# pierluigiferrari/fcn8s_tensorflow

Hardware: AMD Instinct MI355X
Metric: training images/sec at 1024x512 bs16 (higher is better)
Workload: dtype f32; 1 GPU; FCN-8s (VGG-16, fc6 7x7, 20 classes) train step, 1024x512, 16 images/GPU, SGD+momentum, keep_prob 0.5; global_batch=16, parallelism=dp1

## Files before the change

### fcn8s_tensorflow_amd/csrc/fcn8s_internal.h

```cpp
#pragma once
#include <hip/hip_runtime.h>
#include <stdint.h>
#include "../../include/fcn8s_hip.h"

#if defined(__HIP_DEVICE_COMPILE__) && !defined(__gfx950__)
#error "libfcn8s_hip is written for gfx950 (MI355X) only: build with --offload-arch=gfx950"
#endif
#define FCN8S_LDS_BYTES_NEEDED (160u * 1024u)

#include <string>
namespace fcn8s {

extern thread_local const char* g_last_kernel;
void defer_error(int code, const char* fmt, ...) __attribute__((format(printf, 2, 3)));
int take_deferred_error(std::string* text);

struct IgemmArgs {
    const float* x; const float* w; const float* bias; const float* addend; const float* mask;
    float* y;
    int N, Ma, Mb; long long M;
    int Hi, Wi, Cin, ldx;
    int KW, in_scale, tap_step, tap_off, Ktot;
    int Ho, Wo, Cout, ldy;
    int out_scale, out_offy, out_offx;
    int phases_x; long long w_phase_stride;
    float alpha; int relu; float mask_scale;
    int dropout; float keep_prob; unsigned long long seed; unsigned int stream_id;
    int batched; long long x_batch_stride, y_batch_stride;
    int m_fastest;
    int bt, ldw;
    int fixed_tile;
    int split;
};
void launch_igemm(const IgemmArgs& a, int phases, hipStream_t s);

struct Bf16ConvArgs {
    const float* x; const unsigned short* xh;
    const unsigned short* wt; const float* bias; float* y;
    int N, H, W, Cin, Cout, K;
    int relu, dropout; float keep_prob; unsigned long long seed; unsigned int stream_id;
    long long M; int m_fastest;
};
void launch_w_to_bf16_tiles(const float* w, unsigned short* wt, int K, int Cout, hipStream_t s);
bool launch_conv_bf16(const Bf16ConvArgs& a, hipStream_t s);
void launch_f32_to_bf16(const float* x, unsigned short* y, long long n, hipStream_t s);
struct Bf16Conv256Args {
    const unsigned short* xp; const unsigned short* wt; const float* bias; float* y;
    int N, H, W, Cin, Cout, K;
    int relu, dropout; float keep_prob; unsigned long long seed; unsigned int stream_id;
    long long M; int m_fastest;
    const float* addend;
    const float* mask; float mask_scale;
    int any_shape;
    const unsigned short* mask16;
    float* colpart;
    int ksplit; float* part;
    int rows_bn;
    int guarded;
    unsigned short* yb; int yb_pad;
    long long xp_ps, yb_ps, mask16_ps;
};
bool conv_bf16_256_ok(long long M, int Cin, int Cout, int mode);
void launch_w_to_bf16_t(const float* w, unsigned short* wt, int K, int Cout, hipStream_t s);
void launch_f32_to_bf16_padded(const float* x, unsigned short* xp, int N, int H, int W, int C, int pad, hipStream_t s, long long ps = 0);
int conv_bf16_rows_bm(int Cout, int rows_bn);
bool launch_conv_bf16_256(const Bf16Conv256Args& a, hipStream_t s);
struct Fp8ConvArgs {
// ... 220 lines not shown
```

### fcn8s_tensorflow_amd/csrc/igemm.hip

```cpp
#include "fcn8s_internal.h"
#include <cmath>
#include <cstdlib>
#include <map>
#include <mutex>
#include <string>

namespace fcn8s {

thread_local const char* g_last_kernel = nullptr;
#define FCN8S_STR2(x) #x
#define FCN8S_STR(x) FCN8S_STR2(x)

typedef float f32x16 __attribute__((ext_vector_type(16)));
constexpr int BK_ = 16;

static __device__ __forceinline__ float4 ldg4(const float* p) { return *reinterpret_cast<const float4*>(p); }

static __device__ __forceinline__ unsigned xcd_swizzle(unsigned p, unsigned total)
{
    const unsigned q = total >> 3, r = total & 7u, xcd = p & 7u, i = p >> 3;
    return (xcd < r ? xcd * (q + 1) : r * (q + 1) + (xcd - r) * q) + i;
}

thread_local int t_deterministic = 0;
// ... 604 lines not shown
                    float4 v = *reinterpret_cast<const float4*>(&patch[row * LDT + (lane & 7) * 4]);
                    v.x += bv.x; v.y += bv.y; v.z += bv.z; v.w += bv.w;
                    if (mrow + row < p.M) {
                        if (p.mask) {
                            const float4 mk = ldg4(p.mask + (mrow + row) * p.ldy + n0 + wn * TN * 32 + tn * 32 + (lane & 7) * 4);
                            v.x = mk.x > 0.f ? v.x * p.mask_scale : 0.f; v.y = mk.y > 0.f ? v.y * p.mask_scale : 0.f;
                            v.z = mk.z > 0.f ? v.z * p.mask_scale : 0.f; v.w = mk.w > 0.f ? v.w * p.mask_scale : 0.f;
                        }
                        *reinterpret_cast<float4*>(yb + (mrow + row) * p.ldy) = v;
                    }
                }
                __builtin_amdgcn_wave_barrier();
            }
        return;
    }
#pragma unroll
    for (int tn = 0; tn < TN; ++tn) {
        const int col = n0 + wn * TN * 32 + tn * 32 + (lane & 31);
        const float bv = p.bias ? p.bias[col] : 0.f;
#pragma unroll
        for (int tm = 0; tm < TM; ++tm)
#pragma unroll
            for (int r = 0; r < 16; ++r) {
                const long long m = m0 + wm * TM * 32 + tm * 32 + (r & 3) + 8 * (r >> 2) + 4 * (lane >> 5);
                if (m >= p.M) continue;
                const long long off = m * p.ldy;
                float v = acc[tm][tn][r] * p.alpha + bv;
                if (p.addend) v += p.addend[off + col];
                if (p.relu) v = v > 0.f ? v : 0.f;
                if (p.mask) v = p.mask[off + col] > 0.f ? v * p.mask_scale : 0.f;
                if (p.dropout) v = dropout_apply(v, (unsigned long long)(off + col), p.seed, p.stream_id, p.keep_prob);
                Y[off + col] = v;
            }
    }
}

static __device__ __forceinline__ void glds16v(const float* vaddr, unsigned lds_byte_off)
{
    asm volatile("s_mov_b32 m0, %1\n\ts_nop 0\n\tglobal_load_lds_dwordx4 %0, off" ::"v"(vaddr), "s"(lds_byte_off) : "memory", "m0");
}
struct Conv1Args { const float* x4; const float* w48; const float* bias; float* y; const float* zero16; int N, H, W; long long M;
                   unsigned short* yb16; long long yb16_ps; };

__global__ __launch_bounds__(256, 4) void conv1_glds_kernel(const Conv1Args p)
{
    constexpr int BM = 128, BN = 64, BK = 16, NKT = 3, WN = 2, TM = 2, TN = 1, CH = 4, RPI = 16;
    constexpr int A_PW = BM / RPI / 4;
    constexpr int STAGE = BM * BK + BK * BN;
    __shared__ __attribute__((aligned(16))) float smem[NKT * STAGE];
    const int tid = threadIdx.x, lane = tid & 63, wave = __builtin_amdgcn_readfirstlane(tid >> 6);
    const int wm = wave / WN, wn = wave % WN;
    const long long m0 = (long long)blockIdx.x * BM;
    const unsigned lds0 = (unsigned)(size_t)(__attribute__((address_space(3))) float*)smem;
#pragma unroll
    for (int i = 0; i < A_PW; ++i) {
        const int row = (wave * A_PW + i) * RPI + lane / CH, pc = lane % CH;
        const int c = pc ^ ((row >> 2) & 3);
        long long m = m0 + row; if (m >= p.M) m = p.M - 1;
        const int x = (int)(m % p.W); const long long r = m / p.W; const int y = (int)(r % p.H);
#pragma unroll
        for (int kt = 0; kt < NKT; ++kt) {
            const int t = kt * 4 + c, dy = t / 3 - 1, dx = t % 3 - 1;
            const bool ok = t < 9 && (unsigned)(y + dy) < (unsigned)p.H && (unsigned)(x + dx) < (unsigned)p.W;
            const float* src = ok ? p.x4 + (m + (long long)dy * p.W + dx) * 4 : p.zero16;
            glds16v(src, lds0 + (unsigned)(kt * STAGE + (wave * A_PW + i) * 256) * 4u);
        }
// ... 218 lines not shown
                else if (a.split == 2) hipLaunchKernelGGL((gemm_glds_nt_x2_kernel<BM, BN, WM, WN, 3>), grid, dim3(256), 0, s, a);
                else                   hipLaunchKernelGGL((gemm_glds_nt_kernel<BM, BN, WM, WN, 3>), grid, dim3(256), 0, s, a);
                return;
            }
            g_last_kernel = gt[(epi ? 1 : 0) + (a.split == 3 ? 2 : 0)].c_str();
            if (a.split == 3) {
                if (epi) hipLaunchKernelGGL((gemm_glds_x3_kernel<BM, BN, WM, WN, 3, true>), grid, dim3(256), 0, s, a);
                else     hipLaunchKernelGGL((gemm_glds_x3_kernel<BM, BN, WM, WN, 3, false>), grid, dim3(256), 0, s, a);
                return;
            }
            if (a.split == 2) {
                static const std::string x2base = "gemm_glds_x2_kernel<" + std::to_string(BM) + ", " + std::to_string(BN) + ", " + std::to_string(WM) + ", " + std::to_string(WN) + ", 3, ";
                static const std::string x2t[2] = {x2base + "false>", x2base + "true>"};
                g_last_kernel = x2t[epi ? 1 : 0].c_str();
                if (epi) hipLaunchKernelGGL((gemm_glds_x2_kernel<BM, BN, WM, WN, 3, true>), grid, dim3(256), 0, s, a);
                else     hipLaunchKernelGGL((gemm_glds_x2_kernel<BM, BN, WM, WN, 3, false>), grid, dim3(256), 0, s, a);
                return;
            }
            if (epi) hipLaunchKernelGGL((gemm_glds_kernel<BM, BN, WM, WN, 3, true>), grid, dim3(256), 0, s, a);
            else     hipLaunchKernelGGL((gemm_glds_kernel<BM, BN, WM, WN, 3, false>), grid, dim3(256), 0, s, a);
            return;
        }
    }
    if (a.bt) {
        defer_error(FCN8S_ERR_STATE, "transposed-B GEMM (M %lld, K %d, N %d, tile %dx%d) does not fit the LDS-DMA kernel", a.M, a.Ktot, a.Cout, BM, BN);
        return;
    }
    if (mode == 3)      hipLaunchKernelGGL((igemm_fwd_kernel<BM, BN, WM, WN, 3, BKF>), grid, dim3(256), 0, s, a);
    else if (mode == 2) hipLaunchKernelGGL((igemm_fwd_kernel<BM, BN, WM, WN, 2, BKF>), grid, dim3(256), 0, s, a);
    else if (mode == 1) hipLaunchKernelGGL((igemm_fwd_kernel<BM, BN, WM, WN, 1, BKF>), grid, dim3(256), 0, s, a);
    else                hipLaunchKernelGGL((igemm_fwd_kernel<BM, BN, WM, WN, 0, 16>), grid, dim3(256), 0, s, a);
}

void launch_igemm(const IgemmArgs& a, int phases, hipStream_t s)
{
    auto cost = [&](int bm, int bn, int bpc, double eff) {
        const long long blocks = ((a.M + bm - 1) / bm) * ((a.Cout + bn - 1) / bn) * phases;
        const long long n = (blocks + 255) / 256, rem = n % bpc;
        const double tail = rem == 0 ? 0.0 : (rem == 1 ? 2.0 : (rem == 2 ? 2.4 : 3.0));
        return ((double)(n / bpc) * bpc + tail) * bm * bn / eff;
    };
    if (a.fixed_tile && a.Cout % 128 == 0) { launch_igemm_cfg<128, 128, 2, 2>(a, phases, s); return; }
    if (a.fixed_tile && a.Cout % 64 == 0)  { launch_igemm_cfg<128, 64, 2, 2>(a, phases, s); return; }
    if (a.Cout <= 32)      launch_igemm_cfg<128, 32, 4, 1>(a, phases, s);
    else if (a.Cout <= 64) {
        if (cost(128, 64, 4, 1.0) <= cost(64, 64, 4, 0.9)) launch_igemm_cfg<128, 64, 2, 2>(a, phases, s);
        else                                               launch_igemm_cfg<64, 64, 2, 2>(a, phases, s);
    } else {
        const double c128 = cost(128, 128, 3, 1.0), c64x128 = cost(64, 128, 4, 0.9), c64 = cost(64, 64, 4, 0.85);
        if (a.M > 64 && c128 <= c64x128 && c128 <= c64) launch_igemm_cfg<128, 128, 2, 2>(a, phases, s);
        else if (c64x128 <= c64)                        launch_igemm_cfg<64, 128, 2, 2>(a, phases, s);
        else                                            launch_igemm_cfg<64, 64, 2, 2>(a, phases, s);
    }
}

template <int BM, int BN, int WM, int WN, int WK, bool FAST, bool COLSUM>
__global__ __launch_bounds__(256, FAST ? 4 : 1) void wgrad_kernel(const WgradArgs p, const int chunk)
{
    constexpr int BK = 16, LDA = BM, LDB = BN;
    constexpr int TM = BM / WM / 32, TN = BN / WN / 32;
    constexpr int A_F4 = BK * BM / 4, B_F4 = BK * BN / 4;
    constexpr int A_LD = (A_F4 + 255) / 256, B_LD = (B_F4 + 255) / 256;
    static_assert(WM * WN * WK == 4, "4 waves");
    __shared__ __attribute__((aligned(16))) float smem[2 * BK * LDA + 2 * BK * LDB];
    float* As = smem;
    float* Bs = smem + 2 * BK * LDA;

    const int tid = threadIdx.x, lane = tid & 63, wave = tid >> 6;
// ... 848 lines not shown
```

### fcn8s_tensorflow_amd/csrc/model.hip

```cpp
#include "../../include/fcn8s_hip.h"
#include "fcn8s_internal.h"
#include "device_buffer.h"
#include "pass_state.h"
#include <cstdarg>

#include <dlfcn.h>
#include <atomic>
#include <chrono>
#include <thread>
#include <cmath>
#include <cstdio>
#include <cstring>
#include <cstdlib>
#include <algorithm>
#include <mutex>
#include <map>
#include <set>
#include <string>
#include <vector>

using namespace fcn8s;

extern "C" {
typedef struct ncclComm* ncclComm_t;
// ... 60 lines not shown
    std::map<std::string, int> index;
    size_t total = 0;
    size_t bucket_off[FCN8S_MAX_BUCKETS] = {0}, bucket_n[FCN8S_MAX_BUCKETS] = {0};
    hipEvent_t bucket_ev[FCN8S_MAX_BUCKETS] = {nullptr};
    bool bucket_final[FCN8S_MAX_BUCKETS] = {false};
    ncclComm_t comm = nullptr; int comm_rank = 0, comm_world = 1;
    hipStream_t comm_stream = nullptr;
    static constexpr int kCommSlots = FCN8S_MAX_BUCKETS + 1, kCommMisc = FCN8S_MAX_BUCKETS;
    hipEvent_t comm_done[kCommSlots] = {nullptr}; bool comm_pending[FCN8S_MAX_BUCKETS] = {false};
    std::mutex comm_mu;
    std::thread comm_watch; std::atomic<bool> comm_watch_stop{false}, comm_failed{false};
    std::atomic<bool> comm_inflight[kCommSlots] = {}; int64_t comm_enq_ns[kCommSlots] = {0};
    std::string comm_error; int64_t comm_timeout_ms = 600000;
    float *d_params = nullptr, *d_grads = nullptr;
    DeviceBuf<float> own_params, own_grads;
    DeviceBuf<float> d_m, d_v, d_wt, d_w1pad, d_tph[3];
    DeviceBuf<float> d_wino_u; float *d_wino_v = nullptr, *d_wino_m = nullptr;
    size_t ufl = 0;
    int wino_min_cin = 64;
    int wino_tile = 6;
    int wino_fc6 = 1;
    int fc6_fft = 1;
    int fc6_fft_wgrad = 1;
    int wino_tile_hires = 0, wino_hires_pixels = 0;
    int wino_force_tile = 0;
    int precision = FCN8S_PREC_F32;
    bool frozen = false;
    unsigned long long frozen_fp = 0; DeviceBuf<unsigned long long> d_fp;
    PinnedBuf<unsigned long long> h_fp; hipEvent_t fp_event = nullptr;
    std::map<std::string, DeviceBuf<float>> u_cache;
    std::map<std::string, DeviceBuf<float>> u_train;
    bool fwd_train = false;
    PassState pass;
    int deterministic = 0;
    int fuse_dgrad_dout = 1;
    int fuse_out_in = 1;
    int conv1_tiled = 1, conv1_wgrad_mfma = 1;
    int conv1_in_transform = 1;
    DeviceBuf<unsigned short> d_wbf16;
    std::map<std::string, DeviceBuf<unsigned short>> wbf16_cache;
    std::set<std::string> bank_stale; bool banks_stale = false;
    int bf16_gemm256 = 1;
    DeviceBuf<unsigned short> d_abf16;
    std::map<std::string, DeviceBuf<unsigned short>> xbf16;
    using G16Map = std::map<std::string, DeviceBuf<unsigned short>>;
    G16Map xg16, dyg16;
    std::set<std::string> g16_stale;
    int bf16_fuse_pool = 1;
    int bf16_infer_copies = 1;
    int bf16_rows_bn = 0;
    int bf16_acts = 1;
    bool fp8_calibrated = false, fp8_calibrating = false; float fp8_amax[FCN8S_FP8_LAYERS] = {}; DeviceBuf<unsigned> d_fp8_amax;
    std::map<std::string, Q8Buf> q8;
    std::map<std::string, W8Bank> w8; std::set<std::string> w8_valid;
    int saved_wino_min_cin = -1, saved_wino_fc6 = -1;
    int bf16_copy_by_transform = 1;
    int64_t ws_allocs = 0;
    bool x0_ready = false;
    DeviceBuf<char> crf_buf;
    DeviceBuf<char> tta_buf;
    hipStream_t stream = nullptr;
    int64_t step = 0;
    int N = 0, H = 0, W = 0;
    int plan_N = 0;
    DeviceBuf<char> arena;
    std::map<std::string, Act> acts;
// ... 155 lines not shown
            m->groups[k].ev_shared.emplace_back(a, b);
        }
    }
};

static void prof_derived(fcn8s_model* m, const char* what)
{
    if (m && m->profile && m->profile_detail) m->groups[group_id(m, (std::string("derived:") + what).c_str())].launches += 1;
}

struct ConvEpi { float alpha = 1.f; };
struct FwdEpi : ConvEpi {
    const float* bias = nullptr; int relu = 0;
    int dropout = 0; float keep = 1.f; uint32_t stream_id = 0;
    float* pool_out = nullptr; unsigned char* pool_idx = nullptr;
    int skip_y = 0;
    unsigned* relu_bits_out = nullptr;
    unsigned* in_relu_bits_out = nullptr; const char* in_layer = nullptr;
    float* next_v = nullptr; const char* next_layer = nullptr;
};
struct DgradEpi : ConvEpi {
    const float* addend = nullptr;
    const float* mask = nullptr; float mask_scale = 1.f;
    const unsigned* relu_bits_in = nullptr;
    const float* w_fwd = nullptr;
    int lazy_wt = 0;
    float* dm_out = nullptr; const char* dm_out_layer = nullptr;
    const char* yb_layer = nullptr; int yb_K = 3;
    bool yb_only = false;
};

static bool bt_gemm_ok(int K, int N) { return K % 16 == 0 && (N == 64 || N % 128 == 0); }
thread_local int t_op_split = 0;
thread_local int t_op_rows_bn = 0;
thread_local int t_op_planes = 1;
int split_of(const fcn8s_model* m)
{
    if (!m) return t_op_split;
    if (m->precision == FCN8S_PREC_F32X3 || m->precision == FCN8S_PREC_BF16_FWD) return 3;
    if (m->precision == FCN8S_PREC_F32X2 || m->precision == FCN8S_PREC_BF16_FWD_X2) return 2;
    return 0;
}
static inline bool bf16_fwd_mode(const fcn8s_model* m) { return m->precision == FCN8S_PREC_BF16_FWD || m->precision == FCN8S_PREC_BF16_FWD_X2; }
static inline bool bf16_train_mode(const fcn8s_model* m) { return m && m->precision == FCN8S_PREC_BF16_TRAIN; }
static inline long long bf16_guard_rows(int K, int Wp) { return (long long)((K - 1) / 2) * Wp + (K - 1) / 2 + 640; }
#ifndef A_PLANES
#define A_PLANES 1
#endif
static inline long long g16_ps(int N, int H, int W, int K) { const int pad = (K - 1) / 2, Wp_ = W + 2 * pad; return A_PLANES ? ((long long)N * (H + 2 * pad) * Wp_ + 2 * bf16_guard_rows(K, Wp_)) * 32 : 0; }
static inline long long g16_off(long long G, int C) { return A_PLANES ? G * 32 : G * C; }
unsigned short* g16_for(fcn8s_model* m, fcn8s_model::G16Map& bufs, const char* layer, int N, int H, int W, int C, int K, hipStream_t s);
unsigned short* dyb_for(fcn8s_model* m, const char* layer, const float* dy, int N, int H, int W, int C, int K, hipStream_t s, float* db = nullptr, bool* db_done = nullptr);

int wino_tile_for(const fcn8s_model* m, int H, int W, int K = 3)
{
    if (!m || H % 2 || W % 2) return 0;
    if (m->wino_force_tile && K == 3) return (m->wino_force_tile == 6 || (H % m->wino_force_tile == 0 && W % m->wino_force_tile == 0)) ? m->wino_force_tile : 0;
    int tmax = m->wino_tile;
    if (K == 3 && m->wino_tile_hires && m->wino_hires_pixels > 0 && (long long)H * W >= m->wino_hires_pixels && m->wino_tile_hires < tmax) tmax = m->wino_tile_hires;
    const bool t4 = tmax >= 4 && H % 4 == 0 && W % 4 == 0;
    if (K == 7) return (m->wino_tile >= 4 && H % 4 == 0 && W % 4 == 0) ? 4 : 0;
    if (tmax == 6) {
        auto rows = [&](long long tiles) { return m->plan_N == 1 ? (tiles + 63) / 64 * 64 : tiles; };
        const long long c6 = 64LL * rows((long long)((H + 5) / 6) * ((W + 5) / 6)), c4 = t4 ? 36LL * rows((long long)(H / 4) * (W / 4)) : 16LL * rows((long long)(H / 2) * (W / 2));
        if (c6 < c4) return 6;
    }
    return t4 ? 4 : 2;
}
long long wino_tiles(int tile, int N, int H, int W) { return (long long)N * ((H + tile - 1) / tile) * ((W + tile - 1) / tile); }
struct WinoEpi { const float* bias = nullptr; const float* addend = nullptr; const float* mask = nullptr; float mask_scale = 1.f;
                 int relu = 0; int dropout = 0; float keep = 1.f; unsigned long long seed = 0; unsigned int stream_id = 0; float* pool = nullptr; unsigned char* pidx = nullptr;
                 unsigned* rbits_out = nullptr; const unsigned* rbits_in = nullptr; int skip_y = 0;
                 unsigned* in_rbits_out = nullptr;
                 float* next_v = nullptr; bool* fused_out = nullptr; };
static bool fft6_cheaper(const fcn8s_model* m, int H, int W)
// ... 84 lines not shown
    { ProfScope ps(m, "fc6_fft_transform", 0, 4.0 * ((double)N * H * W * Cout + (double)P * T * Cout)); launch_fft_fc6_dout(dz, m->d_wino_m, N, H, W, Cout, s); }
    m->pass.fft6_dyf.give(layer);
    WgradArgs g{}; g.split = 0;
    g.A = xf; g.B = m->d_wino_m; g.C = m->d_wino_u;
    g.N = 1; g.Pa = 1; g.Pb = (int)T; g.P = T;
    g.Ha = 1; g.Wa = (int)T; g.Adim = Cin; g.lda = Cin; g.Areal = Cin;
    g.Bdim = Cout; g.ldb = Cout; g.KW = 1; g.a_scale = 1; g.tap_off = 0; g.ntaps = P; g.ldc = Cout; g.alpha = 1.f; g.colsum = nullptr;
    g.batched = 1; g.a_batch_stride = wino_slab(T, Cin); g.b_batch_stride = wino_slab(T, Cout); g.c_uninitialized = 1;
    { ProfScope ps(m, "fc6_fft_gemm_wgrad", 2.0 * P * T * Cin * Cout, 4.0 * P * (T * (double)(Cin + Cout) + (double)Cin * Cout), layer); launch_wgrad(g, s); }
    { ProfScope ps(m, "fc6_fft_transform", 0, 4.0 * (P + 49.0) * Cin * Cout); launch_fft_fc6_dfilter(m->d_wino_u, dw, Cin, Cout, s); }
    if (db) { ProfScope ps(m, "colsum", 0, 4.0 * N * H * W * Cout); launch_colsum(dz, db, (long long)N * H * W, Cout, s); }
}
static void conv_fft6_dgrad(fcn8s_model* m, const char* layer, const float* dz, const float* uf, float* dx, int N, int H, int W, int Cin, int Cout, hipStream_t s)
{
    const int P = fft_fc6_planes();
    const long long T = fft_fc6_tiles(N, H, W);
    if (!m->pass.fft6_dyf.take(layer)) {
        m->pass.fft6_dyf.drop();
        ProfScope ps(m, "fc6_fft_transform", 0, 4.0 * ((double)N * H * W * Cin + (double)P * T * Cin)); launch_fft_fc6_dout(dz, m->d_wino_m, N, H, W, Cin, s);
    }
    IgemmArgs a = fft6_gemm(m->d_wino_m, uf, m->d_wino_v, T, Cin, Cout);
    a.fixed_tile = 1; a.bt = 1; a.ldw = Cin;
    { ProfScope ps(m, "fc6_fft_gemm_dgrad", 2.0 * P * T * Cin * Cout, 4.0 * P * (T * (double)(Cin + Cout) + (double)Cin * Cout), layer); launch_igemm(a, P, s); }
    { ProfScope ps(m, "fc6_fft_transform", 0, 4.0 * ((double)P * T * Cout + 2.0 * 196.0 * T * Cout + (double)N * H * W * Cout));
      launch_fft_fc6_din(m->d_wino_v, m->d_wino_m, dx, N, H, W, Cout, s); }
}

void conv_winograd(fcn8s_model* m, int tile, int KS, bool fwd, const float* x, const float* wk, float* y, float* u, float* v, float* mm,
                   int N, int H, int W, int Cin, int Cout, const WinoEpi& e, hipStream_t s, const char* layer, bool v_ready = false)
{
    const int P = wino_alpha(tile, KS) * wino_alpha(tile, KS), nsub2 = wino_nsub(KS) * wino_nsub(KS);
    const long long T = wino_tiles(tile, N, H, W);
    const int Kg = nsub2 * Cin;
    IgemmArgs a = fft6_gemm(v, u, mm, T, Kg, Cout); a.split = split_of(m);
    const double tb = 4.0 * ((double)N * H * W * Cin * nsub2 + (double)P * T * Kg), ob = 4.0 * ((double)N * H * W * Cout * ((e.pool ? (e.skip_y ? 0.25 : 1.25) : 1.0) + (e.rbits_in ? 1.0 / 32 : (e.mask ? 1.0 : 0.0)) + (e.addend ? 1.0 : 0.0) + (e.rbits_out ? 1.0 / 32 : 0.0)) + (double)P * T * Cout);
    bool u_cached = false;
    const char* tag = KS == 7 ? (fwd ? "wino_gemm_fc6_fwd" : "wino_gemm_fc6_dgrad") : (fwd ? "wino_gemm_fwd" : "wino_gemm_dgrad");
    if (m && m->frozen && layer && fwd) {
        DeviceBuf<float>& cu = m->u_cache[std::string(layer) + "#" + std::to_string(tile)];
        const std::string key = "u:" + std::string(layer) + "#" + std::to_string(tile);
        if (cu && !m->bank_stale.count(key)) { u = cu; u_cached = true; }
        else if (cu) { u = cu; m->bank_stale.erase(key); }
        else if (cu.grow((size_t)P * Kg * Cout * sizeof(float), s, &m->ws_allocs)) u = cu;
        a.w = u;
    }
    if (m && !u_cached && m->fwd_train && layer && fwd && ((KS == 3 && tile == 6) || (KS == 7 && tile == 4))) {
        DeviceBuf<float>& tu = m->u_train[std::string(layer) + "#" + std::to_string(tile)];
        if (tu.grow((size_t)P * Kg * Cout * sizeof(float), s)) { u = tu; a.w = u; }
    }
    auto pre = [&]() { if (!u_cached) { prof_derived(m, "wino_filter_kernel"); launch_wino_filter(tile, wk, u, Cin, Cout, KS, s); } if (!v_ready) launch_wino_input(tile, x, v, N, H, W, Cin, KS, s, e.in_rbits_out); };
    auto post = [&]() {
        if (e.next_v && tile == 6 && KS == 3 && e.relu && e.bias && !e.addend && !e.mask && !e.dropout && !e.pool && !e.rbits_in &&
            launch_wino_out_in(mm, e.bias, e.next_v, e.rbits_out, N, H, W, Cout, s, m && m->fuse_out_in >= 2)) { if (e.fused_out) *e.fused_out = true; return; }
        launch_wino_output(tile, mm, e.bias, e.addend, e.mask, e.mask_scale, e.relu, (e.skip_y && e.pool) ? nullptr : y, N, H, W, Cout, e.dropout, e.keep, e.seed, e.stream_id, s, e.pool, e.pidx, KS, e.rbits_out, e.rbits_in); };
    const double ob_fused = 4.0 * (2.0 * P * T * Cout + (e.rbits_out ? (double)N * H * W * Cout / 32 : 0.0));
    { ProfScope ps(m, "wino_transform", 0, (v_ready ? 0.0 : tb) + (u_cached ? 0.0 : (double)(KS * KS + P * nsub2) * 4 * Cin * Cout)); pre(); }
    { ProfScope ps(m, tag, 2.0 * P * T * Kg * Cout, 4.0 * P * (T * (double)(Kg + Cout) + (double)Kg * Cout), layer); launch_igemm(a, P, s); }
    { ProfScope ps(m, "wino_transform", 0, ob); post(); if (e.fused_out && *e.fused_out && m && m->profile && !m->groups.empty()) { const int g = group_id(m, "wino_transform"); m->groups[g].bytes += ob_fused - ob; } }
}

static void conv_direct(fcn8s_model* m, const char* group, IgemmArgs a, const float* x, const float* w, float* y,
                        int N, int H, int W, int Cin, int Cout, int K, hipStream_t s, int real_cin, const char* layer)
{
    a.split = split_of(m);
    a.x = x; a.w = w; a.y = y;
    a.N = N; a.Ma = H; a.Mb = W; a.M = (long long)N * H * W;
    a.Hi = H; a.Wi = W; a.Cin = Cin; a.ldx = Cin;
// ... 76 lines not shown
              done = launch_conv_bf16_256(g, s); }
            if (done) {
                if (g.yb) m->pass.dyg16_filled.insert(e.yb_layer);
                if (g.colpart) {
                    ProfScope ps(m, "colsum", 0, 4.0 * prow * Cout);
                    launch_colsum(g.colpart, Gp(m, std::string(e.yb_layer) + "/biases"), prow, Cout, s);
                    m->pass.db_taken.insert(e.yb_layer); m->pass.dy_bf16_only.insert(e.yb_layer);
                }
                return;
            }
            if (g.colpart) { defer_error(FCN8S_ERR_SHAPE, "bf16_train: %s's data gradient was refused by the flat-position kernel", layer); return; }
        }
    }
    if (bf16_step && m->pass.dy_bf16_only.count(layer)) {
        defer_error(FCN8S_ERR_SHAPE, "bf16_train: %s's data gradient could not run on the bf16 kernel and its fp32 output gradient was not kept (option \"bf16_acts\" = 0 keeps it)", layer); return;
    }
    if (bf16_step && e.mask && m->pass.in_bf16_only.count(layer)) {
        defer_error(FCN8S_ERR_SHAPE, "bf16_train: %s's data gradient could not run on the bf16 kernel and its fp32 mask was not kept (option \"bf16_acts\" = 0 keeps it)", layer); return;
    }
    const bool dm_ready = m && m->pass.dm.take(layer), v_ready = m && m->pass.dgrad_v.take(layer);
    if (m) m->pass.drop_backward_handoffs();
    if (m && K == 7 && layer && e.alpha == 1.f && !e.addend && !e.mask && !e.relu_bits_in) {
        auto kept = m->u_train.find(std::string(layer) + "#fft");
        if (m->pass.fft6_ready.holds(layer) && kept != m->u_train.end() && kept->second && fft6_on(m, N, H, W, Cout, Cin) && bt_gemm_ok(Cin, Cout)) {
            conv_fft6_dgrad(m, layer, x, kept->second, y, N, H, W, Cin, Cout, s);
            return;
        }
    }
    const bool wino3 = m && K == 3 && m->wino_min_cin > 0 && Cin >= m->wino_min_cin && m->d_wino_v && wino_tile_for(m, H, W, 3);
    const bool wino7 = m && K == 7 && m->wino_fc6 && m->d_wino_v && wino_tile_for(m, H, W, 7) == 4;
    if (wino3 && dm_ready && e.w_fwd && wino_tile_for(m, H, W, 3) == 6 && Cin % 64 == 0 && Cout % 64 == 0 && e.alpha == 1.f) {
        const int P = 64;
        const long long T = wino_tiles(6, N, H, W);
        IgemmArgs a = fft6_gemm(m->d_wino_m, m->d_wino_u, m->d_wino_v, T, Cin, Cout); a.split = split_of(m);
        auto kept = m->u_train.find(std::string(layer) + "#6");
        if (kept != m->u_train.end() && kept->second && bt_gemm_ok(Cin, Cout)) {
            a.w = kept->second; a.bt = 1; a.ldw = Cin;
        } else {
            ProfScope ps(m, "wino_transform", 0, (double)(9 + P) * 4 * Cin * Cout); launch_wino_filter(6, e.w_fwd, m->d_wino_u, Cout, Cin, 3, s, 1);
        }
        { ProfScope ps(m, "wino_gemm_dgrad", 2.0 * P * T * Cin * Cout, 4.0 * P * (T * (double)(Cin + Cout) + (double)Cin * Cout), layer); launch_igemm(a, P, s); }
        if (e.dm_out && e.dm_out_layer && e.relu_bits_in && !e.addend && e.mask_scale == 1.f) {
            ProfScope ps(m, "wino_transform", 0, 4.0 * ((double)N * H * W * Cout / 32 + 2.0 * P * T * Cout));
            launch_wino_dgrad_output_dout(m->d_wino_v, e.relu_bits_in, e.dm_out, N, H, W, Cout, s);
            m->pass.dm_prefilled.give(e.dm_out_layer);
            return;
        }
        { ProfScope ps(m, "wino_transform", 0, 4.0 * ((double)N * H * W * Cout * (1.0 + (e.relu_bits_in ? 1.0 / 32 : (e.mask ? 1.0 : 0.0)) + (e.addend ? 1.0 : 0.0)) + (double)P * T * Cout));
          launch_wino_dgrad_output(m->d_wino_v, e.addend, e.mask, e.mask_scale, e.relu_bits_in, y, N, H, W, Cout, s); }
        return;
    }
    if (wino7 && dm_ready && e.alpha == 1.f && !e.mask && !e.addend && bt_gemm_ok(Cin, 4 * Cout)) {
        auto kept = m->u_train.find(std::string(layer) + "#4");
        if (kept != m->u_train.end() && kept->second) {
            const int P = 49, Ng = 4 * Cout;
            const long long T = wino_tiles(4, N, H, W);
            IgemmArgs a = fft6_gemm(m->d_wino_m, kept->second, m->d_wino_v, T, Cin, Ng); a.split = split_of(m);
            a.bt = 1; a.ldw = Cin;
            { ProfScope ps(m, "wino_gemm_fc6_dgrad", 2.0 * P * T * Cin * Ng, 4.0 * P * (T * (double)(Cin + Ng) + (double)Cin * Ng), layer); launch_igemm(a, P, s); }
            { ProfScope ps(m, "wino_transform", 0, 4.0 * ((double)N * H * W * Cout + (double)P * T * Ng)); launch_wino_dgrad_output_sub44(m->d_wino_v, y, N, H, W, Cout, s); }
            return;
        }
    }
    if (e.lazy_wt && e.w_fwd) {
        ProfScope ps(m, "weight_relayout", 0, 8.0 * K * K * Cin * Cout); launch_flip_transpose(e.w_fwd, const_cast<float*>(w), K * K, Cout, Cin, s);
    }
    if ((wino3 || wino7) && Cin % 16 == 0 && Cout % 64 == 0 && e.alpha == 1.f) {
// ... 1366 lines not shown
    if (!m->fp8_calibrated) return FCN8S_ERR_STATE;
    memcpy(amax, m->fp8_amax, sizeof m->fp8_amax);
    return FCN8S_OK;
}
int fcn8s_fp8_set_calibration(fcn8s_model* m, const float* amax, int n)
{
    if (!m || !amax) return fail(m, FCN8S_ERR_BAD_ARG, "fcn8s_fp8_set_calibration: null argument");
    if (n != FCN8S_FP8_LAYERS) return fail(m, FCN8S_ERR_BAD_ARG, "fcn8s_fp8_set_calibration: needs FCN8S_FP8_LAYERS (14) maxima");
    for (int i = 0; i < n; ++i)
        if (!std::isfinite(amax[i]) || amax[i] < 0.f) return fail(m, FCN8S_ERR_BAD_ARG, "fcn8s_fp8_set_calibration: maxima must be finite and >= 0");
    memcpy(m->fp8_amax, amax, sizeof m->fp8_amax);
    m->fp8_calibrated = true;
    return FCN8S_OK;
}

static int* model_option(fcn8s_model* m, const std::string& key)
{
    if (key == "winograd_min_cin") return &m->wino_min_cin;
    if (key == "winograd_tile") return &m->wino_tile;
    if (key == "winograd_fc6") return &m->wino_fc6;
    if (key == "fc6_fft") return &m->fc6_fft;
    if (key == "fc6_fft_wgrad") return &m->fc6_fft_wgrad;
    if (key == "tconv_gemm") return &m->tconv_gemm;
    if (key == "fuse_dgrad_dout") return &m->fuse_dgrad_dout;
    if (key == "fuse_out_in") return &m->fuse_out_in;
    if (key == "bf16_gemm256") return &m->bf16_gemm256;
    if (key == "winograd_tile_hires") return &m->wino_tile_hires;
    if (key == "winograd_hires_pixels") return &m->wino_hires_pixels;
    if (key == "conv1_tiled") return &m->conv1_tiled;
    if (key == "conv1_wgrad_mfma") return &m->conv1_wgrad_mfma;
    if (key == "bf16_copy_by_transform") return &m->bf16_copy_by_transform;
    if (key == "conv1_in_transform") return &m->conv1_in_transform;
    if (key == "deterministic") return &m->deterministic;
    if (key == "bf16_acts") return &m->bf16_acts;
    if (key == "bf16_rows_bn") return &m->bf16_rows_bn;
    if (key == "keep_output_gradients") return &m->keep_dy;
    if (key == "bf16_infer_copies") return &m->bf16_infer_copies;
    if (key == "bf16_fuse_pool") return &m->bf16_fuse_pool;
    return nullptr;
}
int fcn8s_set_option(fcn8s_model* m, const char* key, int64_t value)
{
    if (!key) return fail(m, FCN8S_ERR_BAD_ARG, "fcn8s_set_option: null key");
    const std::string k = key;
    if (k == "device_bytes_live") return fail(m, FCN8S_ERR_BAD_ARG, "fcn8s_set_option: 'device_bytes_live' is read-only");
    if (!m) {
        if (k == "op_f32x3") { t_op_split = value ? 3 : 0; return FCN8S_OK; }
        if (k == "op_deterministic") { t_deterministic = value ? 1 : 0; return FCN8S_OK; }
        if (k == "op_bf16_planes") { t_op_planes = value ? 1 : 0; return FCN8S_OK; }
        if (k == "op_bf16_rows_bn") { if (value != 0 && value != 64 && value != 128) return fail(nullptr, FCN8S_ERR_BAD_ARG, "op_bf16_rows_bn must be 0, 64 or 128"); t_op_rows_bn = (int)value; return FCN8S_OK; }
        if (k == "op_split_pieces") {
            if (value != 0 && value != 2 && value != 3) return fail(nullptr, FCN8S_ERR_BAD_ARG, "fcn8s_set_option: op_split_pieces is 0, 2 or 3");
            t_op_split = (int)value; return FCN8S_OK;
        }
        return fail(nullptr, FCN8S_ERR_NOT_FOUND, "fcn8s_set_option: unknown op-context option '" + k + "' (model options need a model)");
    }
    if (k == "workspace_allocations" || k == "frozen") return fail(m, FCN8S_ERR_BAD_ARG, "fcn8s_set_option: '" + k + "' is read-only (the frozen state is set with fcn8s_freeze_params)");
    if (k == "comm_timeout_ms") {
        if (value < 1) return fail(m, FCN8S_ERR_BAD_ARG, "comm_timeout_ms must be >= 1");
        std::lock_guard<std::mutex> lk(m->comm_mu); m->comm_timeout_ms = value; return FCN8S_OK;
    }
    if (k == "conv1_tiled" || k == "conv1_wgrad_mfma" || k == "bf16_copy_by_transform" || k == "conv1_in_transform" || k == "deterministic" || k == "bf16_acts" || k == "bf16_rows_bn" || k == "bf16_fuse_pool" || k == "keep_output_gradients" || k == "bf16_infer_copies") {
        *model_option(m, k) = k == "bf16_rows_bn" ? (int)value : (value ? 1 : 0);
        return FCN8S_OK;
    }
    int* slot = model_option(m, k);
    if (!slot) return fail(m, FCN8S_ERR_NOT_FOUND, "fcn8s_set_option: unknown option '" + k + "'");
    if (direct_mode(m->precision) && (k == "winograd_min_cin" || k == "winograd_fc6")) {
        if (value < 0) return fail(m, FCN8S_ERR_BAD_ARG, "fcn8s_set_option: negative value");
        (k == "winograd_min_cin" ? m->saved_wino_min_cin : m->saved_wino_fc6) = (int)value;
        return FCN8S_OK;
    }
    if (k == "winograd_tile" && value != 2 && value != 4 && value != 6) return fail(m, FCN8S_ERR_BAD_ARG, "winograd_tile must be 2, 4 or 6");
    if (k == "winograd_tile_hires" && value != 0 && value != 2 && value != 4 && value != 6) return fail(m, FCN8S_ERR_BAD_ARG, "winograd_tile_hires must be 0, 2, 4 or 6");
    if (k == "winograd_min_cin" && value < 0) return fail(m, FCN8S_ERR_BAD_ARG, "winograd_min_cin must be >= 0 (0 = direct convolution everywhere)");
    if (k == "fuse_out_in" && (value < 0 || value > 2)) return fail(m, FCN8S_ERR_BAD_ARG, "fuse_out_in must be 0, 1 or 2");
    if (k == "fc6_fft_wgrad" && (value < 0 || value > 2)) return fail(m, FCN8S_ERR_BAD_ARG, "fc6_fft_wgrad must be 0, 1 or 2");
    if (*slot == (int)value) return FCN8S_OK;
    HIPCHK(m, hipStreamSynchronize(m->stream));
    *slot = (k == "winograd_fc6" || k == "fc6_fft" || k == "tconv_gemm") ? (value != 0) : (int)value;
    drop_arena(m);
    drop_banks(m, true); m->u_train.clear();
    return FCN8S_OK;
}
int fcn8s_get_option(const fcn8s_model* m, const char* key, int64_t* value)
{
    if (!key || !value) return FCN8S_ERR_BAD_ARG;
    const std::string k = key;
    if (k == "device_bytes_live") { *value = g_device_bytes_live.load(); return FCN8S_OK; }
    if (!m) {
        if (k == "op_f32x3") { *value = t_op_split == 3; return FCN8S_OK; }
        if (k == "op_deterministic") { *value = t_deterministic; return FCN8S_OK; }
        if (k == "op_bf16_planes") { *value = t_op_planes; return FCN8S_OK; }
        if (k == "op_bf16_rows_bn") { *value = t_op_rows_bn; return FCN8S_OK; }
        if (k == "op_split_pieces") { *value = t_op_split; return FCN8S_OK; }
        return FCN8S_ERR_NOT_FOUND;
    }
    if (k == "comm_timeout_ms") { *value = m->comm_timeout_ms; return FCN8S_OK; }
    if (k == "workspace_allocations") { *value = m->ws_allocs; return FCN8S_OK; }
    if (k == "frozen") { *value = m->frozen ? 1 : 0; return FCN8S_OK; }
    const int* slot = model_option(const_cast<fcn8s_model*>(m), k);
    if (!slot) return FCN8S_ERR_NOT_FOUND;
    *value = *slot;
    if (direct_mode(m->precision) && k == "winograd_min_cin" && m->saved_wino_min_cin >= 0) *value = m->saved_wino_min_cin;
    if (direct_mode(m->precision) && k == "winograd_fc6" && m->saved_wino_fc6 >= 0) *value = m->saved_wino_fc6;
    return FCN8S_OK;
}

int fcn8s_set_stream(fcn8s_model* m, void* s) { if (!m) return FCN8S_ERR_BAD_ARG; m->stream = (hipStream_t)s; return FCN8S_OK; }
int fcn8s_synchronize(fcn8s_model* m) { if (!m) return FCN8S_ERR_BAD_ARG; HIPCHK(m, hipStreamSynchronize(m->stream)); return FCN8S_OK; }

int fcn8s_num_params(const fcn8s_model* m) { return m ? (int)m->params.size() : 0; }
int fcn8s_param_info(const fcn8s_model* m, int i, const char** name, int32_t* ndim, int64_t shape[4], int64_t* off)
{
    if (!m || i < 0 || i >= (int)m->params.size()) return FCN8S_ERR_BAD_ARG;
    const ParamInfo& p = m->params[i];
    if (name) *name = p.name.c_str();
    if (ndim) *ndim = p.ndim;
    if (shape) for (int k = 0; k < 4; ++k) shape[k] = p.shape[k];
    if (off) *off = (int64_t)p.offset;
    return FCN8S_OK;
}
int fcn8s_param_index(const fcn8s_model* m, const char* name)
{
    if (!m || !name) return -1;
// ... 1243 lines not shown
{
    if (Cin % 4 || Cout % 4 || K % 2 == 0) return fail(nullptr, FCN8S_ERR_BAD_ARG, "conv2d: Cin, Cout must be multiples of 4 and K odd");
    FwdEpi e; e.bias = bias; e.relu = relu;
    conv_fwd(nullptr, "", x, w, y, N, H, W, Cin, Cout, K, e, (hipStream_t)stream);
    OPCHK(); return FCN8S_OK;
}

int fcn8s_op_conv2d_winograd(void* stream, const float* x, const float* w, const float* bias, float* y,
                             int N, int H, int W, int Cin, int Cout, int K, int relu, int tile)
{
    if ((tile != 2 && tile != 4 && tile != 6) || (K != 3 && K != 7) || (K == 7 && tile != 4) || Cin % 16 || Cout % 32 || (tile != 6 && (H % tile || W % tile)) || H % 2 || W % 2)
        return fail(nullptr, FCN8S_ERR_BAD_ARG, "conv2d_winograd: needs tile in {2,4,6} (4 for K = 7), K in {3,7}, Cin % 16, Cout % 32, even H and W (multiples of tile for tile 2 and 4)");
    hipStream_t s = (hipStream_t)stream;
    const size_t T = (size_t)wino_tiles(tile, N, H, W), P = (size_t)wino_alpha(tile, K) * wino_alpha(tile, K), Kg = (size_t)wino_nsub(K) * wino_nsub(K) * Cin;
    DeviceBuf<float> u, v, mm;
    if (!u.grow(P * Kg * Cout * 4, s) || !v.grow(P * (size_t)wino_slab(T, (int)Kg) * 4, s) || !mm.grow(P * (size_t)wino_slab(T, Cout) * 4, s)) return fail(nullptr, FCN8S_ERR_OOM, "hipMalloc");
    WinoEpi we; we.bias = bias; we.relu = relu;
    conv_winograd(nullptr, tile, K, true, x, w, y, u, v, mm, N, H, W, Cin, Cout, we, s, nullptr);
    hipStreamSynchronize(s);
    OPCHK(); return FCN8S_OK;
}

int fcn8s_op_conv3x3_winograd_fwd_bwd(void* stream, const float* x, const float* w, const float* bias, const float* dy, const float* dx_addend,
                                      float* y, float* pool, float* dx, float* dw, float* db,
                                      int N, int H, int W, int Cin, int Cout, int tile, int pooled, int mask_mode)
{
    if ((tile != 2 && tile != 4 && tile != 6) || Cin % 64 || Cout % 64 || H % 2 || W % 2 || (tile != 6 && (H % tile || W % tile)) || !x || !w || !dy || !dx || !dw ||
        (pooled && (!pool || tile < 4)) || (!pooled && !y) || mask_mode < 0 || mask_mode > 2)
        return fail(nullptr, FCN8S_ERR_BAD_ARG, "conv3x3_winograd_fwd_bwd: needs tile in {2,4,6}, Cin % 64 == 0, Cout % 64 == 0, even H and W (multiples of tile for tiles 2, 4), "
                                                "pooled only with tiles 4 and 6, mask_mode in {0,1,2}");
    hipStream_t s = (hipStream_t)stream;
    fcn8s_model mm; fcn8s_model* m = &mm;
    m->stream = s; m->wino_min_cin = 16; m->wino_tile = 6; m->wino_force_tile = tile; m->N = N; m->H = H; m->W = W;
    m->precision = t_op_split == 3 ? FCN8S_PREC_F32X3 : t_op_split == 2 ? FCN8S_PREC_F32X2 : FCN8S_PREC_F32;
    const int al = tile + 2, P = al * al, cmax = std::max(Cin, Cout);
    const size_t T = (size_t)wino_tiles(tile, N, H, W);
    const size_t slab_max = (size_t)P * (size_t)wino_slab((long long)T, cmax), slab_in = (size_t)P * (size_t)wino_slab((long long)T, Cin);
    DeviceBuf<float> wino_v, wino_m, wv, wt, pidx, rbits;
    bool ok = true;
    auto dalloc = [&](DeviceBuf<float>& b, size_t nfloats) { ok = ok && b.grow(nfloats * sizeof(float), s); };
    dalloc(m->d_wino_u, (size_t)P * cmax * cmax); dalloc(wino_v, slab_max); dalloc(wino_m, slab_max);
    dalloc(wv, slab_in); dalloc(wt, (size_t)9 * Cin * Cout);
    if (pooled) dalloc(pidx, ((size_t)N * (H / 2) * (W / 2) * Cout + 3) / 4);
    if (mask_mode == 2) dalloc(rbits, wino_rbits_words(tile, N, H, W, Cin));
    if (!ok) return fail(nullptr, FCN8S_ERR_OOM, "hipMalloc");
    m->d_wino_v = wino_v; m->d_wino_m = wino_m;
    Act a; a.p = wv; a.n = slab_in; m->acts["wv:op"] = a;
    m->fwd_train = true; m->train_mode = true;
    { FwdEpi e; e.bias = bias; e.relu = 1;
      if (pooled) { e.pool_out = pool; e.pool_idx = (unsigned char*)pidx.get(); e.skip_y = y == nullptr; }
      if (mask_mode == 2) { e.in_relu_bits_out = (unsigned*)rbits.get(); e.in_layer = "prev"; }
      conv_fwd(m, "op", x, w, y, N, H, W, Cin, Cout, 3, e, s, 0, "op"); }
    hipMemsetAsync(dw, 0, (size_t)9 * Cin * Cout * sizeof(float), s);
    if (db) hipMemsetAsync(db, 0, (size_t)Cout * sizeof(float), s);
    conv_wgrad(m, "op", x, dy, dw, db, N, H, W, Cin, Cout, 3, 1.f, s, 0, "op", tile >= 4, pooled ? (const unsigned char*)pidx.get() : nullptr);
    { DgradEpi e; e.w_fwd = w; e.lazy_wt = 1; e.addend = dx_addend;
      if (mask_mode) { e.mask = x; e.mask_scale = 1.f; }
      if (mask_mode == 2 && m->pass.rbits_ok.count("prev")) e.relu_bits_in = (const unsigned*)rbits.get();
      conv_dgrad(m, "op", dy, wt, dx, N, H, W, Cout, Cin, 3, e, s, "op"); }
    hipStreamSynchronize(s);
    OPCHK(); return FCN8S_OK;
}

int fcn8s_op_conv7x7_fc6_fwd_bwd(void* stream, const float* x, const float* w, const float* bias, const float* dy,
                                 float* y, float* dx, float* dw, float* db,
                                 int N, int H, int W, int Cin, int Cout, int path, float keep_prob, uint64_t seed, int* dft_products)
// ... 351 lines not shown
```

Before: 298.2 images/sec.

## Add persistent warp-specialized streaming GEMM for Winograd batched small-K GEMMs

```diff
diff --git a/fcn8s_tensorflow_amd/csrc/fcn8s_internal.h b/fcn8s_tensorflow_amd/csrc/fcn8s_internal.h
--- a/fcn8s_tensorflow_amd/csrc/fcn8s_internal.h
+++ b/fcn8s_tensorflow_amd/csrc/fcn8s_internal.h
@@ -31,8 +31,13 @@
     int bt, ldw;
     int fixed_tile;
     int split;
+    int stream_gemm;
 };
 void launch_igemm(const IgemmArgs& a, int phases, hipStream_t s);
+bool stream_gemm_eligible(const IgemmArgs& a, int phases);
+unsigned stream_gemm_grid(const IgemmArgs& a, int phases, int option, int block_cap);
+extern thread_local int t_stream_gemm_blocks;
+extern thread_local long long t_stream_gemm_launches;
 
 struct Bf16ConvArgs {
     const float* x; const unsigned short* xh;
diff --git a/fcn8s_tensorflow_amd/csrc/igemm.hip b/fcn8s_tensorflow_amd/csrc/igemm.hip
--- a/fcn8s_tensorflow_amd/csrc/igemm.hip
+++ b/fcn8s_tensorflow_amd/csrc/igemm.hip
@@ -660,6 +660,141 @@
                 if (p.dropout) v = dropout_apply(v, (unsigned long long)(off + col), p.seed, p.stream_id, p.keep_prob);
                 Y[off + col] = v;
             }
+    }
+}
+
+static __device__ __forceinline__ void glds16s(const float* sbase, unsigned voff, unsigned lds_byte_off)
+{
+    asm volatile("s_nop 4\n\ts_mov_b32 m0, %2\n\ts_nop 0\n\tglobal_load_lds_dwordx4 %0, %1" ::"v"(voff), "s"(sbase), "s"(lds_byte_off) : "memory", "m0");
+}
+constexpr int stream_gemm_bm(int K, int N) { return (K == 128 && N == 64) ? 64 : 4096 / K; }
+static __host__ __device__ constexpr int stream_gemm_sw(int row) { return ((row & 7) << 1) | ((row >> 3) & 1); }
+template <int K, int N, bool BT>
+__global__ __launch_bounds__(320, 3) void gemm_stream_kernel(const IgemmArgs p, const unsigned ntm, const unsigned total)
+{
+    constexpr int BM = stream_gemm_bm(K, N), NKT = K / 16, STAGE = BM * K;
+    constexpr int CPR = K / 4, RPI = 64 / CPR;
+    constexpr int NT = 16384 / STAGE, IPT = BM / RPI;
+    constexpr int WN = N / 32, WM = 4 / WN, TM = BM / WM / 32, LDT = 36;
+    static_assert((K == 64 || K == 128) && (N == 64 || N == 128) && TM >= 1 && BM == WM * TM * 32 && (NT == 2 || NT == 4) && (NT - 2) * IPT <= 63, "shapes");
+    __shared__ __attribute__((aligned(16))) float smem[NT * STAGE + 4 * 16 * LDT];
+    const int tid = threadIdx.x, lane = tid & 63, wave = __builtin_amdgcn_readfirstlane(tid >> 6);
+    const unsigned it0 = (unsigned)((unsigned long long)total * blockIdx.x / gridDim.x);
+    const unsigned it1 = (unsigned)((unsigned long long)total * (blockIdx.x + 1) / gridDim.x);
+
+    if (wave == 4) {
+        const unsigned lds0 = (unsigned)(size_t)(__attribute__((address_space(3))) float*)smem;
+        const int lrow = lane / CPR, pc = lane % CPR;
+        unsigned voff_full[IPT];
+#pragma unroll
+        for (int i = 0; i < IPT; ++i) { const int r = i * RPI + lrow; voff_full[i] = (unsigned)(r * p.ldx + (pc ^ stream_gemm_sw(r)) * 4) * 4u; }
+        auto issue = [&](unsigned item, unsigned slot) {
+            const unsigned z = item / ntm;
+            const long long m0 = (long long)(item - z * ntm) * BM;
+            const float* xb = p.x + (long long)z * p.x_batch_stride + m0 * p.ldx;
+            const unsigned l0 = lds0 + slot * (unsigned)(STAGE * 4);
+            if (m0 + BM <= p.M) {
+#pragma unroll
+                for (int i = 0; i < IPT; ++i) glds16s(xb, voff_full[i], l0 + i * 1024u);
+            } else {
+#pragma unroll
+                for (int i = 0; i < IPT; ++i) {
+                    const int r = i * RPI + lrow;
+                    long long m = m0 + r; if (m >= p.M) m = p.M - 1;
+                    glds16s(xb, (unsigned)((m - m0) * p.ldx + (pc ^ stream_gemm_sw(r)) * 4) * 4u, l0 + i * 1024u);
+                }
+            }
+        };
+#pragma unroll
+        for (unsigned t = 0; t < NT - 1; ++t)
+            if (it0 + t < it1) issue(it0 + t, t);
+        for (unsigned it = it0; it < it1; ++it) {
+            const unsigned ahead = it1 - 1 - it < NT - 2 ? it1 - 1 - it : NT - 2;
+            if (NT == 4 && ahead == 2) wait_vmcnt<2 * IPT>(); else if (NT == 4 && ahead == 1) wait_vmcnt<IPT>(); else wait_vmcnt<0>();
+            __builtin_amdgcn_s_barrier();
+            if (it + NT - 1 < it1) issue(it + NT - 1, (it + NT - 1 - it0) & (NT - 1));
+        }
+        return;
+    }
+
+    const int wm = wave / WN, wn = wave % WN, half = lane >> 5, l31 = lane & 31;
+    int a_off[TM], a_sw[TM];
+#pragma unroll
+    for (int tm = 0; tm < TM; ++tm) {
+        const int row = wm * TM * 32 + tm * 32 + l31;
+        a_off[tm] = row * K;
+        a_sw[tm] = stream_gemm_sw(row);
+    }
+    float* patch = smem + NT * STAGE + wave * 16 * LDT;
+    float b[NKT][2][4];
+    const unsigned b_lane = (unsigned)(half * 4 * N + wn * 32 + l31), bt_lane = (unsigned)((wn * 32 + l31) * p.ldw + half * 4);
+    for (unsigned it = it0; it < it1;) {
+        const unsigned z = it / ntm;
+        const unsigned zend = (z + 1) * ntm < it1 ? (z + 1) * ntm : it1;
+        {
+            const float* Wp = p.w + (long long)z * p.w_phase_stride;
+#pragma unroll
+            for (int kt = 0; kt < NKT; ++kt)
+#pragma unroll
+                for (int kk2 = 0; kk2 < 2; ++kk2) {
+                    if (BT) {
+                        const float4 t = ldg4(Wp + (kt * 16 + kk2 * 8) + bt_lane);
+                        b[kt][kk2][0] = t.x; b[kt][kk2][1] = t.y; b[kt][kk2][2] = t.z; b[kt][kk2][3] = t.w;
+                    } else {
+#pragma unroll
+                        for (int j = 0; j < 4; ++j) b[kt][kk2][j] = (Wp + (kt * 16 + kk2 * 8 + j) * N)[b_lane];
+                    }
+                }
+#pragma unroll
+            for (int kt = 0; kt < NKT; ++kt)
+#pragma unroll
+                for (int kk2 = 0; kk2 < 2; ++kk2)
+#pragma unroll
+                    for (int j = 0; j < 4; ++j) asm volatile("" : "+v"(b[kt][kk2][j]));
+        }
+        for (; it < zend; ++it) {
+        __builtin_amdgcn_s_barrier();
+        const long long m0 = (long long)(it - z * ntm) * BM;
+        f32x16 acc[TM];
+#pragma unroll
+        for (int tm = 0; tm < TM; ++tm)
+#pragma unroll
+            for (int r = 0; r < 16; ++r) acc[tm][r] = 0.f;
+        const float* sa = smem + ((it - it0) & (NT - 1)) * STAGE;
+#pragma unroll
+        for (int kt = 0; kt < NKT; ++kt)
+#pragma unroll
+            for (int kk2 = 0; kk2 < 2; ++kk2) {
+                float4 af[TM];
+#pragma unroll
+                for (int tm = 0; tm < TM; ++tm)
+                    af[tm] = *reinterpret_cast<const float4*>(sa + a_off[tm] + (((kt * 4 + kk2 * 2 + half) ^ a_sw[tm]) * 4));
+#pragma unroll
+                for (int j = 0; j < 4; ++j)
+#pragma unroll
+                    for (int tm = 0; tm < TM; ++tm) {
+                        const float av = j == 0 ? af[tm].x : j == 1 ? af[tm].y : j == 2 ? af[tm].z : af[tm].w;
+                        acc[tm] = __builtin_amdgcn_mfma_f32_32x32x2f32(av, b[kt][kk2][j], acc[tm], 0, 0, 0);
+                    }
+            }
+        float* Y = p.y + (long long)z * p.y_batch_stride + wn * 32 + (lane & 7) * 4;
+#pragma unroll
+        for (int tm = 0; tm < TM; ++tm)
+#pragma unroll
+            for (int h = 0; h < 2; ++h) {
+#pragma unroll
+                for (int r = 0; r < 8; ++r) patch[((r & 3) + 8 * (r >> 2) + 4 * half) * LDT + l31] = acc[tm][h * 8 + r];
+                __builtin_amdgcn_wave_barrier();
+#pragma unroll
+                for (int j = 0; j < 2; ++j) {
+                    const int row = j * 8 + (lane >> 3);
+                    const float4 v = *reinterpret_cast<const float4*>(&patch[row * LDT + (lane & 7) * 4]);
+                    const long long m = m0 + wm * TM * 32 + tm * 32 + h * 16 + row;
+                    if (m < p.M) *reinterpret_cast<float4*>(Y + m * p.ldy) = v;
+                }
+                __builtin_amdgcn_wave_barrier();
+            }
+        }
     }
 }
 
@@ -944,8 +1079,62 @@
     else                hipLaunchKernelGGL((igemm_fwd_kernel<BM, BN, WM, WN, 0, 16>), grid, dim3(256), 0, s, a);
 }
 
+thread_local int t_stream_gemm_blocks = 0;
+thread_local long long t_stream_gemm_launches = 0;
+bool stream_gemm_eligible(const IgemmArgs& a, int phases)
+{
+    if (!a.batched || a.split != 0 || phases < 1 || a.M < 1) return false;
+    if ((a.Ktot != 64 && a.Ktot != 128) || (a.Cout != 64 && a.Cout != 128) || a.Ktot != a.Cin) return false;
+    if (a.bias || a.addend || a.mask || a.relu || a.dropout || a.alpha != 1.f) return false;
+    if (a.out_scale != 1 || a.in_scale != 1 || a.tap_off != 0 || a.out_offy != 0 || a.out_offx != 0) return false;
+    if (a.ldx < a.Ktot || a.ldx % 4 != 0 || a.ldy < a.Cout || a.ldy % 4 != 0 || (long long)127 * a.ldx >= (1LL << 29)) return false;
+    if (a.bt && (a.ldw < a.Ktot || a.ldw % 4 != 0 || (long long)127 * a.ldw >= (1LL << 29))) return false;
+    const int BM = stream_gemm_bm(a.Ktot, a.Cout);
+    return ((a.M + BM - 1) / BM) * phases < (1LL << 31);
+}
+constexpr int kStreamGrid = 512, kStreamMinItems = 64;
+static bool stream_gemm_shape_wins(int K, int N, int bt) { return bt ? true : (K == 64 && N == 128); }
+unsigned stream_gemm_grid(const IgemmArgs& a, int phases, int option, int block_cap)
+{
+    if (option <= 0 || !stream_gemm_eligible(a, phases)) return 0;
+    const int BM = stream_gemm_bm(a.Ktot, a.Cout);
+    const long long total = ((a.M + BM - 1) / BM) * phases;
+    if (option == 1 && (!stream_gemm_shape_wins(a.Ktot, a.Cout, a.bt) || total < (long long)kStreamGrid * kStreamMinItems)) return 0;
+    long long g = total < kStreamGrid ? total : kStreamGrid;
+    if (block_cap > 0 && g > block_cap) g = block_cap;
+    return (unsigned)g;
+}
+template <int K, int N, bool BT>
+static void launch_gemm_stream_cfg(const IgemmArgs& a, unsigned grid, unsigned ntm, unsigned total, hipStream_t s)
+{
+    static const std::string tag = "gemm_stream_kernel<" + std::to_string(K) + ", " + std::to_string(N) + ", " + (BT ? "true>" : "false>");
+    g_last_kernel = tag.c_str();
+    hipLaunchKernelGGL((gemm_stream_kernel<K, N, BT>), dim3(grid), dim3(320), 0, s, a, ntm, total);
+}
+static bool launch_gemm_stream(const IgemmArgs& a, int phases, hipStream_t s)
+{
+    const unsigned grid = stream_gemm_grid(a, phases, a.stream_gemm, t_stream_gemm_blocks);
+    if (!grid) return false;
+    const int BM = stream_gemm_bm(a.Ktot, a.Cout);
+    const unsigned ntm = (unsigned)((a.M + BM - 1) / BM), total = ntm * (unsigned)phases;
+    const int sel = (a.Ktot == 128 ? 4 : 0) + (a.Cout == 128 ? 2 : 0) + (a.bt ? 1 : 0);
+    switch (sel) {
+    case 0: launch_gemm_stream_cfg<64, 64, false>(a, grid, ntm, total, s); break;
+    case 1: launch_gemm_stream_cfg<64, 64, true>(a, grid, ntm, total, s); break;
+    case 2: launch_gemm_stream_cfg<64, 128, false>(a, grid, ntm, total, s); break;
+    case 3: launch_gemm_stream_cfg<64, 128, true>(a, grid, ntm, total, s); break;
+    case 4: launch_gemm_stream_cfg<128, 64, false>(a, grid, ntm, total, s); break;
+    case 5: launch_gemm_stream_cfg<128, 64, true>(a, grid, ntm, total, s); break;
+    case 6: launch_gemm_stream_cfg<128, 128, false>(a, grid, ntm, total, s); break;
+    default: launch_gemm_stream_cfg<128, 128, true>(a, grid, ntm, total, s); break;
+    }
+    ++t_stream_gemm_launches;
+    return true;
+}
+
 void launch_igemm(const IgemmArgs& a, int phases, hipStream_t s)
 {
+    if (a.stream_gemm && launch_gemm_stream(a, phases, s)) return;
     auto cost = [&](int bm, int bn, int bpc, double eff) {
         const long long blocks = ((a.M + bm - 1) / bm) * ((a.Cout + bn - 1) / bn) * phases;
         const long long n = (blocks + 255) / 256, rem = n % bpc;
diff --git a/fcn8s_tensorflow_amd/csrc/model.hip b/fcn8s_tensorflow_amd/csrc/model.hip
--- a/fcn8s_tensorflow_amd/csrc/model.hip
+++ b/fcn8s_tensorflow_amd/csrc/model.hip
@@ -116,6 +116,7 @@
     std::map<std::string, DeviceBuf<float>> u_train;
     bool fwd_train = false;
     PassState pass;
+    int stream_gemm = 1;
     int deterministic = 0;
     int fuse_dgrad_dout = 1;
     int fuse_out_in = 1;
@@ -337,6 +338,7 @@
 
 static bool bt_gemm_ok(int K, int N) { return K % 16 == 0 && (N == 64 || N % 128 == 0); }
 thread_local int t_op_split = 0;
+thread_local int t_op_stream_gemm = 1;
 thread_local int t_op_rows_bn = 0;
 thread_local int t_op_planes = 1;
 int split_of(const fcn8s_model* m)
@@ -346,6 +348,7 @@
     if (m->precision == FCN8S_PREC_F32X2 || m->precision == FCN8S_PREC_BF16_FWD_X2) return 2;
     return 0;
 }
+int stream_of(const fcn8s_model* m) { return m ? m->stream_gemm : t_op_stream_gemm; }
 static inline bool bf16_fwd_mode(const fcn8s_model* m) { return m->precision == FCN8S_PREC_BF16_FWD || m->precision == FCN8S_PREC_BF16_FWD_X2; }
 static inline bool bf16_train_mode(const fcn8s_model* m) { return m && m->precision == FCN8S_PREC_BF16_TRAIN; }
 static inline long long bf16_guard_rows(int K, int Wp) { return (long long)((K - 1) / 2) * Wp + (K - 1) / 2 + 640; }
@@ -496,7 +499,7 @@
     const int P = wino_alpha(tile, KS) * wino_alpha(tile, KS), nsub2 = wino_nsub(KS) * wino_nsub(KS);
     const long long T = wino_tiles(tile, N, H, W);
     const int Kg = nsub2 * Cin;
-    IgemmArgs a = fft6_gemm(v, u, mm, T, Kg, Cout); a.split = split_of(m);
+    IgemmArgs a = fft6_gemm(v, u, mm, T, Kg, Cout); a.split = split_of(m); a.stream_gemm = stream_of(m);
     const double tb = 4.0 * ((double)N * H * W * Cin * nsub2 + (double)P * T * Kg), ob = 4.0 * ((double)N * H * W * Cout * ((e.pool ? (e.skip_y ? 0.25 : 1.25) : 1.0) + (e.rbits_in ? 1.0 / 32 : (e.mask ? 1.0 : 0.0)) + (e.addend ? 1.0 : 0.0) + (e.rbits_out ? 1.0 / 32 : 0.0)) + (double)P * T * Cout);
     bool u_cached = false;
     const char* tag = KS == 7 ? (fwd ? "wino_gemm_fc6_fwd" : "wino_gemm_fc6_dgrad") : (fwd ? "wino_gemm_fwd" : "wino_gemm_dgrad");
@@ -639,7 +642,7 @@
     if (wino3 && dm_ready && e.w_fwd && wino_tile_for(m, H, W, 3) == 6 && Cin % 64 == 0 && Cout % 64 == 0 && e.alpha == 1.f) {
         const int P = 64;
         const long long T = wino_tiles(6, N, H, W);
-        IgemmArgs a = fft6_gemm(m->d_wino_m, m->d_wino_u, m->d_wino_v, T, Cin, Cout); a.split = split_of(m);
+        IgemmArgs a = fft6_gemm(m->d_wino_m, m->d_wino_u, m->d_wino_v, T, Cin, Cout); a.split = split_of(m); a.stream_gemm = stream_of(m);
         auto kept = m->u_train.find(std::string(layer) + "#6");
         if (kept != m->u_train.end() && kept->second && bt_gemm_ok(Cin, Cout)) {
             a.w = kept->second; a.bt = 1; a.ldw = Cin;
@@ -2072,6 +2075,7 @@
     if (key == "bf16_copy_by_transform") return &m->bf16_copy_by_transform;
     if (key == "conv1_in_transform") return &m->conv1_in_transform;
     if (key == "deterministic") return &m->deterministic;
+    if (key == "stream_gemm") return &m->stream_gemm;
     if (key == "bf16_acts") return &m->bf16_acts;
     if (key == "bf16_rows_bn") return &m->bf16_rows_bn;
     if (key == "keep_output_gradients") return &m->keep_dy;
@@ -2087,6 +2091,9 @@
     if (!m) {
         if (k == "op_f32x3") { t_op_split = value ? 3 : 0; return FCN8S_OK; }
         if (k == "op_deterministic") { t_deterministic = value ? 1 : 0; return FCN8S_OK; }
+        if (k == "op_stream_gemm") { if (value < 0 || value > 2) return fail(nullptr, FCN8S_ERR_BAD_ARG, "op_stream_gemm must be 0, 1 or 2"); t_op_stream_gemm = (int)value; return FCN8S_OK; }
+        if (k == "op_stream_gemm_blocks") { if (value < 0 || value > (1 << 20)) return fail(nullptr, FCN8S_ERR_BAD_ARG, "op_stream_gemm_blocks must be 0 (the launcher's grid) or a block count"); t_stream_gemm_blocks = (int)value; return FCN8S_OK; }
+        if (k == "op_stream_gemm_launches") return fail(nullptr, FCN8S_ERR_BAD_ARG, "fcn8s_set_option: 'op_stream_gemm_launches' is read-only");
         if (k == "op_bf16_planes") { t_op_planes = value ? 1 : 0; return FCN8S_OK; }
         if (k == "op_bf16_rows_bn") { if (value != 0 && value != 64 && value != 128) return fail(nullptr, FCN8S_ERR_BAD_ARG, "op_bf16_rows_bn must be 0, 64 or 128"); t_op_rows_bn = (int)value; return FCN8S_OK; }
         if (k == "op_split_pieces") {
@@ -2099,6 +2106,10 @@
     if (k == "comm_timeout_ms") {
         if (value < 1) return fail(m, FCN8S_ERR_BAD_ARG, "comm_timeout_ms must be >= 1");
         std::lock_guard<std::mutex> lk(m->comm_mu); m->comm_timeout_ms = value; return FCN8S_OK;
+    }
+    if (k == "stream_gemm") {
+        if (value < 0 || value > 2) return fail(m, FCN8S_ERR_BAD_ARG, "stream_gemm must be 0, 1 or 2");
+        m->stream_gemm = (int)value; return FCN8S_OK;
     }
     if (k == "conv1_tiled" || k == "conv1_wgrad_mfma" || k == "bf16_copy_by_transform" || k == "conv1_in_transform" || k == "deterministic" || k == "bf16_acts" || k == "bf16_rows_bn" || k == "bf16_fuse_pool" || k == "keep_output_gradients" || k == "bf16_infer_copies") {
         *model_option(m, k) = k == "bf16_rows_bn" ? (int)value : (value ? 1 : 0);
@@ -2131,6 +2142,9 @@
     if (!m) {
         if (k == "op_f32x3") { *value = t_op_split == 3; return FCN8S_OK; }
         if (k == "op_deterministic") { *value = t_deterministic; return FCN8S_OK; }
+        if (k == "op_stream_gemm") { *value = t_op_stream_gemm; return FCN8S_OK; }
+        if (k == "op_stream_gemm_blocks") { *value = t_stream_gemm_blocks; return FCN8S_OK; }
+        if (k == "op_stream_gemm_launches") { *value = t_stream_gemm_launches; return FCN8S_OK; }
         if (k == "op_bf16_planes") { *value = t_op_planes; return FCN8S_OK; }
         if (k == "op_bf16_rows_bn") { *value = t_op_rows_bn; return FCN8S_OK; }
         if (k == "op_split_pieces") { *value = t_op_split; return FCN8S_OK; }
@@ -3440,6 +3454,7 @@
     hipStream_t s = (hipStream_t)stream;
     fcn8s_model mm; fcn8s_model* m = &mm;
     m->stream = s; m->wino_min_cin = 16; m->wino_tile = 6; m->wino_force_tile = tile; m->N = N; m->H = H; m->W = W;
+    m->stream_gemm = t_op_stream_gemm;
     m->precision = t_op_split == 3 ? FCN8S_PREC_F32X3 : t_op_split == 2 ? FCN8S_PREC_F32X2 : FCN8S_PREC_F32;
     const int al = tile + 2, P = al * al, cmax = std::max(Cin, Cout);
     const size_t T = (size_t)wino_tiles(tile, N, H, W);
```

New measurement: 297.9 images/sec. No clear change (-0.1%).
